# nannau/DoWnGAN

Measured on AMD Instinct MI355X. Metric: train-step samples/sec (G+D+GP), higher is better.
Workload: dtype bf16

## Files before the change

### downgan_amd/_lib.py

```python
from __future__ import annotations

import ctypes as C
import os

_HERE = os.path.dirname(os.path.abspath(__file__))
LIB_PATH = os.environ.get("DG_LIB_OVERRIDE") or os.path.join(_HERE, "csrc", "libdowngan_hip.so")

DG_F32, DG_BF16 = 0, 1
STATUS = {0: "DG_OK", -1: "DG_ERR_BAD_SHAPE", -2: "DG_ERR_BAD_DTYPE", -3: "DG_ERR_BAD_ARG", -4: "DG_ERR_LAUNCH"}


class Epilogue(C.Structure):
    _fields_ = [("bias", C.c_void_p), ("has_act", C.c_int), ("act_slope", C.c_float),
                ("r1", C.c_void_p), ("ldr1", C.c_int64), ("s1", C.c_float),
                ("r2", C.c_void_p), ("ldr2", C.c_int64), ("s2", C.c_float),
                ("mask", C.c_void_p), ("ldmask", C.c_int64), ("mask_slope", C.c_float),
                ("accumulate", C.c_int), ("mask_bits", C.c_void_p), ("out_bits", C.c_void_p),
                ("mask_c0", C.c_int), ("mask_last", C.c_int), ("out_q", C.c_void_p), ("out_qs", C.c_void_p), ("ldqs", C.c_int64),
                ("out_u", C.c_void_p), ("out_ue", C.c_void_p), ("skip_y", C.c_int), ("out_amax", C.c_void_p)]


class ConvGeom(C.Structure):
    _fields_ = [("dtype", C.c_int), ("N", C.c_int), ("H", C.c_int), ("W", C.c_int),
                ("Cin", C.c_int), ("Cout", C.c_int), ("stride", C.c_int), ("cin_real", C.c_int), ("pixel_shuffle", C.c_int),
# ... 113 lines not shown
                ("nbins", C.c_int), ("below", C.c_int * TEMPORAL_MAX_THR), ("lag", C.c_int * TEMPORAL_MAX_LAGS),
                ("scale", C.c_float * EOF_MAX_C), ("offset", C.c_float * EOF_MAX_C),
                ("thr", (C.c_float * TEMPORAL_MAX_THR) * HIST_MAX_OUT), ("lo", (C.c_float * TEMPORAL_MAX_LAGS) * HIST_MAX_OUT),
                ("inv_w", (C.c_float * TEMPORAL_MAX_LAGS) * HIST_MAX_OUT)]


MINMAX_PARTS = 256
_vp, _i, _i64, _f = C.c_void_p, C.c_int, C.c_int64, C.c_float
_PROTOS = {
    "dg_conv3x3_fwd": [C.POINTER(ConvGeom), C.POINTER(Epilogue), _vp, _vp, _vp, _vp],
    "dg_conv3x3_dgrad": [C.POINTER(ConvGeom), C.POINTER(Epilogue), _vp, _vp, _vp, _vp],
    "dg_conv3x3_wgrad": [C.POINTER(ConvGeom), _vp, _vp, _vp, _vp, _vp],
    "dg_conv3x3_wgrad_dense": [_vp, _i, _vp, _vp, _vp, _vp, _vp],
    "dg_conv3x3_wgrad_f8": [C.POINTER(ConvGeom), _vp, _vp, _vp, _vp, _vp, _vp],
    "dg_exp_from_amax": [_vp, _i, _i, _vp, _vp],
    "dg_conv3x3_wgrad_dense_f8": [C.POINTER(ConvGeom), _i, _vp, _vp, _vp, _vp, _vp, _vp],
    "dg_gather_gemm": [C.POINTER(GGDesc), C.POINTER(Epilogue), _vp, _vp, _vp, _vp],
    "dg_conv3x3_plan": [C.POINTER(ConvGeom), _i, C.POINTER(GGDesc)],
    "dg_last_conv_kernels": [],
    "dg_last_wgrad_kernel": [],
    "dg_conv3x3_dgrad_launches": [C.POINTER(ConvGeom)],
    "dg_conv3x3_dgrad_stream_eligible": [C.POINTER(ConvGeom), C.POINTER(Epilogue)],
    "dg_set_s2_dgrad_stream": [C.c_int],
    "dg_colsum": [_i, _vp, _i64, _i64, _i64, _i64, _i, _vp, _vp],
    "dg_colsum_multi": [_i, _vp, _i64, _i64, _i, _i, _vp, _vp],
    "dg_repack_conv_weights": [_i, _i, _vp, _vp, _i, _i, _vp],
    "dg_repack_dense_dgrad": [_i, _vp, _i, _i, _vp, _vp],
    "dg_wgrad_unswap": [_vp, _vp, _i, _i, _vp],
    "dg_linear_fwd": [_i, _vp, _i64, _vp, _i64, _vp, _i, _i, _i, _i64, _vp],
    "dg_linear_dx": [_i, _i, _vp, _i, _vp, _i64, _vp, _i64, _vp, _i64, _f, _i, _i, _i64, _vp],
    "dg_linear_dw": [_i, _vp, _i, _vp, _i64, _vp, _i64, _i, _i, _i64, _vp],
    "dg_linear_dw_wide": [_i, _vp, _i, _vp, _i64, _vp, _i64, _i, _i, _i64, _i, _vp],
    "dg_bias_act": [_i, _vp, _i, _vp, _vp, _i, _i, _i, _i, _f, _vp, _i, _f, _vp],
    "dg_mask_mul": [_i, _vp, _i64, _vp, _i64, _i64, _i, _f, _vp],
    "dg_axpby": [_i, _vp, _i64, _vp, _i64, _f, _vp, _i64, _f, _i64, _i, _vp],
    "dg_gp_interp": [_i, _vp, _vp, _vp, _vp, _i, _i64, _vp],
    "dg_gp_interp_c2": [_i, _vp, _vp, _i64, _vp, _vp, _vp, _vp, _i, _i64, _vp],
    "dg_scale_rows_c2": [_i, _vp, _i64, _vp, _vp, _i, _i64, _vp],
    "dg_sumsq_rows": [_i, _vp, _i, _i64, _vp, _vp],
    "dg_gp_finish": [_vp, _i, _i, _f, _f, _vp, _vp, _vp],
    "dg_scale_rows": [_i, _vp, _vp, _vp, _i, _i64, _vp],
    "dg_l1": [_i, _vp, _i64, _vp, _i64, _i64, _i, _vp, _vp, _i64, _f, _vp, _i64, _vp],
    "dg_sqdiff": [_i, _vp, _i64, _vp, _i64, _i64, _i, _vp, _vp],
    "dg_sum_strided": [_vp, _i, _i, _f, _vp, _vp],
    "dg_fill_col": [_vp, _i, _i, _i, _f, _vp],
    "dg_adam": [_vp, _vp, _vp, _vp, _vp, _i64, _f, _f, _f, _f, _i, _f, _vp],
# ... 137 lines not shown
```

### downgan_amd/csrc/conv_plan.hip

```cpp
#include "gg_common.h"

thread_local int g_last_kinds = 0;

static int gg_validate(const dg_gg_desc* d, bool f8 = false, bool compact_src = false) {
  if (d->dtype != DG_F32 && d->dtype != DG_BF16) return DG_ERR_BAD_DTYPE;
  const int epc = f8 ? 16 : d->dtype == DG_F32 ? 4 : 8;
  if (d->N <= 0 || d->Hs <= 0 || d->Ws <= 0 || d->Hg <= 0 || d->Wg <= 0 || d->Hd <= 0 || d->Wd <= 0) return DG_ERR_BAD_SHAPE;
  if (d->Cred <= 0 || d->Cred % 8 || d->Nout <= 0 || d->Nout % 16) return DG_ERR_BAD_SHAPE;
  if (d->ntaps < 1 || d->ntaps > 9) return DG_ERR_BAD_SHAPE;
  if ((compact_src ? d->lds % 2 || d->lds < 2 : d->lds % epc) || d->ldd % 4 || d->ldw % epc) return DG_ERR_BAD_SHAPE;
  for (int t = 0; t < d->ntaps; ++t) {
    if (d->tap_dy[t] < -1 || d->tap_dy[t] > 1 || d->tap_dx[t] < -1 || d->tap_dx[t] > 1) return DG_ERR_BAD_ARG;
    if (d->tap_w[t] < 0 || d->tap_w[t] > 8) return DG_ERR_BAD_ARG;
  }
  if (d->src_ps && ((d->Cred / 4) % 8)) return DG_ERR_BAD_SHAPE;
  if (d->dst_ps && ((d->Nout / 4) % 16)) return DG_ERR_BAD_SHAPE;
  if ((long long)d->N * d->Hg * d->Wg >= (1ll << 31)) return DG_ERR_BAD_SHAPE;
  if (d->dst_ps) {
    if (2 * d->Hg > d->Hd || 2 * d->Wg > d->Wd) return DG_ERR_BAD_SHAPE;
  } else {
    if ((d->Hg - 1) * d->dy_mul + d->dy_off >= d->Hd || (d->Wg - 1) * d->dx_mul + d->dx_off >= d->Wd) return DG_ERR_BAD_SHAPE;
    if (d->dy_off < 0 || d->dx_off < 0 || d->dy_mul < 1 || d->dx_mul < 1) return DG_ERR_BAD_SHAPE;
  }
  return DG_OK;
// ... 232 lines not shown
  int n = dg_conv3x3_plan(g, 1, d);
  if (n < 0) return n;
  dg_gg_desc ds;
  if (seg_dgrad_desc(d, n, &ds) && ds.Cred % 128 == 0) {
    ds.lds = q->ldxq;
    return gather_gemm_impl(&ds, ep, q->xq, q->wq, dx, stream, false, q, true);
  }
  for (int i = 0; i < n; ++i) {
    d[i].lds = q->ldxq;
    int rc = gather_gemm_impl(&d[i], ep, q->xq, q->wq, dx, stream, false, q);
    if (rc) return rc;
  }
  return DG_OK;
}

extern "C" int dg_last_conv_kernels(void) { return g_last_kinds; }

extern "C" int dg_conv3x3_dgrad_stream_eligible(const dg_conv_geom* g, const dg_epilogue* ep) {
  const int rc = geom_validate(g);
  if (rc) return rc;
  return s2dgrad_stream_eligible(g, ep) ? 1 : 0;
}

extern "C" int dg_conv3x3_dgrad_launches(const dg_conv_geom* g) {
  dg_gg_desc d[4], ds;
  const int n = dg_conv3x3_plan(g, 1, d);
  if (n < 0) return n;
  return seg_dgrad_desc(d, n, &ds) ? 1 : n;
}
```

### downgan_amd/csrc/conv_s2dgrad.hip

```cpp
#include "gg_common.h"

namespace {

constexpr int NT = 512;
constexpr int RING_PIX = 17;
constexpr int RING_PITCH = 288;
constexpr int MASK_OFF = RING_PIX * RING_PITCH;
constexpr int RING_ROW = MASK_OFF + 2 * 32 * 16;
constexpr int RING_CHUNKS = RING_PIX * 16;

struct S2DArgs {
  const char* dy; const char* w; char* dx; const char* mask_bits;
  float slope;
  int Ho, Wo;
  int nstrips, nitems, trips;
};

__device__ __forceinline__ __amdgpu_buffer_rsrc_t uniform_rsrc(const char* p) {
  const unsigned long long b = (unsigned long long)p;
  const unsigned long long u = ((unsigned long long)(unsigned)__builtin_amdgcn_readfirstlane((int)(unsigned)(b >> 32)) << 32) |
                               (unsigned)__builtin_amdgcn_readfirstlane((int)(unsigned)b);
  return __builtin_amdgcn_make_buffer_rsrc((void*)u, 0, (int)DG_OOB_OFF, 0x00020000);
}

template <bool MASK>
__device__ __forceinline__ void store_pixel(const f32x4_t& f0, const f32x4_t& f1, unsigned mb, float slope, __amdgpu_buffer_rsrc_t rY,
                                            unsigned off) {
  float v[8] = {f0[0], f0[1], f0[2], f0[3], f1[0], f1[1], f1[2], f1[3]};
  if (MASK) {
    unsigned sh = mb << 24;
    const float one = 1.f;
#pragma unroll
    for (int e = 7; e >= 0; --e) {
      float f;
      asm("v_add_co_u32_e32 %1, vcc, %1, %1\n\tv_cndmask_b32_e32 %0, %2, %3, vcc" : "=&v"(f), "+v"(sh) : "v"(slope), "v"(one) : "vcc");
      v[e] *= f;
    }
  }
  u32x4_t t;
#pragma unroll
  for (int k = 0; k < 4; ++k) t[k] = pack_bf16x2(v[2 * k], v[2 * k + 1]);
  __builtin_amdgcn_raw_buffer_store_b128(t, rY, off, 0, 0);
}

template <bool MASK, bool C11>
__device__ __forceinline__ void s2d_run(const S2DArgs& a, char* ring) {
  constexpr int NTAP = C11 ? 4 : 5;
  const int tid = threadIdx.x, lane = tid & 63, q = (tid >> 6) & 3;
  const int l15 = lane & 15, g = lane >> 4;

  uint4 wr[NTAP * 8];
  {
    constexpr int TW11[4] = {0, 2, 6, 8}, TWX[5] = {4, 3, 5, 1, 7};
#pragma unroll
    for (int cb = 0; cb < 2; ++cb)
#pragma unroll
      for (int t = 0; t < NTAP; ++t)
#pragma unroll
        for (int kk = 0; kk < 2; ++kk)
#pragma unroll
          for (int j = 0; j < 2; ++j) {
            const int n = 32 * q + 8 * (l15 >> 2) + 4 * j + (l15 & 3);
            const int tw = C11 ? TW11[t] : TWX[t];
            wr[((cb * NTAP + t) * 2 + kk) * 2 + j] =
                *reinterpret_cast<const uint4*>(a.w + ((long long)n * 1152 + tw * 128 + 64 * cb + 32 * kk + 8 * g) * 2);
          }
// ... 178 lines not shown
```

### downgan_amd/csrc/gg_common.h

```cpp
#pragma once
#include "dg_internal.h"

#include <stdlib.h>
#include <type_traits>


extern thread_local int g_last_kinds;

struct GGArgs {
  const void* x; const void* w; void* y;
  const float* bias; const void* r1; const void* r2; const void* mask;
  const void* mask_bits; void* out_bits;
  void* out_q; void* out_qs;
  void* out_u; const unsigned char* out_ue;
  int no_y;
  unsigned* out_amax;
  int ldqs, qs_shift;
  long long ldx, ldw, ldy, ldr1, ldr2, ldmask;
  int M, Hg, Wg, Hs, Ws;
  int cch, kchunks, Cred, ntaps;
  int sy_mul, sx_mul;
  unsigned long long tap_lo; unsigned tap_hi;
  int Nout, Hd, Wd, dy_mul, dx_mul, dy_off, dx_off;
  int src_ps, dst_ps, cps_src_chunks, cps_dst;
// ... 480 lines not shown
      case 2305: run(std::integral_constant<int, 2305>{}, htag); break;
      case 2312: run(std::integral_constant<int, 2312>{}, htag); break;
      case 2328: run(std::integral_constant<int, 2328>{}, htag); break;
      case 2336: run(std::integral_constant<int, 2336>{}, htag); break;
      case 258: run(std::integral_constant<int, 258>{}, htag); break;
      case 261: run(std::integral_constant<int, 261>{}, htag); break;
      case 2306: run(std::integral_constant<int, 2306>{}, htag); break;
      case 2309: run(std::integral_constant<int, 2309>{}, htag); break;
      case 4353: run(std::integral_constant<int, 4353>{}, htag); break;
      case 4354: run(std::integral_constant<int, 4354>{}, htag); break;
      case 4357: run(std::integral_constant<int, 4357>{}, htag); break;
      case 6402: run(std::integral_constant<int, 6402>{}, htag); break;
      case 6405: run(std::integral_constant<int, 6405>{}, htag); break;
      default: run(std::integral_constant<int, -1>{}, htag); break;
    }
  };
  dispatch(std::integral_constant<int, 0>{});
  EPI_STAMP(2);
  if constexpr (NH == 2) dispatch(std::integral_constant<int, 1>{});
  EPI_STAMP(3);
#undef EPI_STAMP
}

struct F8Args { const unsigned char* xs; const unsigned char* ws; int ldxs; };

int gg_launch_rows(GGArgs& a, int dtype, hipStream_t st);
bool gg_regroup_taps_by_plane(GGArgs& a);
bool gg_halo_row_step_ok(long long Ws, long long ldx, int dtype, int mult);
int gg_launch_halo(GGArgs& a, int dtype, int N, bool s2, bool ps, int nw, hipStream_t st);
int gg_launch_halo_f8(GGArgs& a, const F8Args& f, int N, bool s2, int nw, hipStream_t st);
int gg_launch_halo16(GGArgs& a, int dtype, int N, hipStream_t st);
int gg_launch_im2col(GGArgs& a, int dtype, hipStream_t st);
bool s2dgrad_stream_eligible(const dg_conv_geom* g, const dg_epilogue* ep);
int s2dgrad_stream_mode();
int s2dgrad_stream_launch(const dg_conv_geom* g, const dg_epilogue* ep, const void* dy, const void* w, void* dx, hipStream_t st);
```

### downgan_amd/engine.py

```python
from __future__ import annotations

import dataclasses
import math
import os

import torch

from . import layout
from .ops import Conv

G_SLOPE = 0.01
C_SLOPE = 0.2
RES_SCALE = 0.2
FC_HID = 100
FC_HID_P = 112
FC_HID_LD = 128
FC_OUT_P = 16


@dataclasses.dataclass
class HyperParams:
    gp_lambda: float = 10.0
    critic_iterations: int = 5
    batch_size: int = 32
# ... 132 lines not shown
        self.c_pad = [layout.pad16(c) for c in self.c_real]
        self.convs = []
        h = fine_dim
        for l, st in enumerate(self.STRIDES):
            self.convs.append(Conv(batch, h, h, self.c_pad[l], self.c_pad[l + 1], st, False,
                                   cin_real=(nc if l == 0 and nc <= 2 else 0), net="C",
                                   cin_alg=self.c_real[l], cout_alg=self.c_real[l + 1]))
            h //= st
        self.hf = h
        self.fc_k = h * h * self.c_pad[8]
        P = self.P = ParamStore(ops)
        for l, cv in enumerate(self.convs):
            P.add(f"features.{2 * l}.weight", (cv.Cout, 9, cv.Cin))
            P.conv_dgrad[f"features.{2 * l}.weight"] = (cv.Cout, cv.Cin)
        P.add("features.0.bias", (self.c_pad[1],))
        P.add("classifier.0.weight", (FC_HID_P, self.fc_k))
        P.add("classifier.0.bias", (FC_HID_LD,))
        P.add("classifier.2.weight", (FC_OUT_P, FC_HID_LD))
        P.add("classifier.2.bias", (FC_OUT_P,))
        P.finalize()
        o = ops
        use_bits = os.environ.get("DG_NO_MASK_BITS") is None and all(c >= 128 and c % 64 == 0 for c in self.c_pad[1:])
        self.f8 = bool(getattr(o, "f8", False))
        self.stacked = bool(stacked) and use_bits and not self.f8 and 3 * batch <= 128 and os.environ.get("DG_NO_FC1_FUSED") is None
        self.stack_from = (int(stacked) - 1 if (stacked is not True and int(stacked) > 1) else 0) if self.stacked else 0
        cap = 3 * batch if self.stacked else batch
        self.cap = cap
        full = lambda cv: (cap,) + tuple(o.out_shape(cv))[1:]
        self._acts_all = [o.zeros(*full(cv)) for cv in self.convs[:7]] + [None]
        self._us_all = [o.zeros(*full(cv)) for cv in self.convs]
        self._bits_all = [o.zeros(*o.bits_shape(full(cv)), dtype=torch.int16) for cv in self.convs] if use_bits else None
        self.acts = [a[:batch] if a is not None else o.zeros(*o.out_shape(self.convs[7])) for a in self._acts_all]
        self.us = [u[:batch] for u in self._us_all]
        self.act_bits = [b[:batch] for b in self._bits_all] if use_bits else None
        self._h1pre_all = o.zeros(cap, FC_HID_LD, dtype=torch.float32)
        self._h1_all = o.zeros(cap, FC_HID_LD)
        self._outpre_all = o.zeros(cap, FC_OUT_P, dtype=torch.float32)
        self._out_all = o.zeros(cap, FC_OUT_P, dtype=torch.float32)
        self._dout_all = o.zeros(cap, FC_OUT_P, dtype=torch.float32)
        self.uh1 = o.zeros(batch, FC_HID_LD, dtype=torch.float32)
        self._cv_cache = {}
        self._tan = self._th1pre = self._th1 = self._ones = None
        self.fc1_fused = 3 * batch <= 128 and os.environ.get("DG_NO_FC1_FUSED") is None
        if self.fc1_fused:
            self._y7_all = o.zeros(4 * batch, *self.acts[7].shape[1:])
            self._uh1_all = o.zeros(3 * batch, FC_HID_LD, dtype=torch.float32)
# ... 85 lines not shown
        o, P = self.ops, self.P
        if self.fc1_fused:
            s = 3 if fc1_slot is None else fc1_slot
            self.acts[7] = self._y7_all[s * self.B:(s + 1) * self.B]
        cur = x
        want_u = self.f8 and for_wgrad and self._act_exp_ok
        self._u_act_live = want_u
        l0u = self.l0u and self._act_exp_ok
        for l, cv in enumerate(self.convs):
            f8kw = dict(xq=self.actq[l - 1] if l else None, wq=self.wq_f[l], out_q=self.actq[l]) if self.f8 else {}
            if want_u and self.actu[l] is not None:
                f8kw["out_u"] = self.actu[l]
            if l0u and l == 0:
                f8kw = dict(out_u=self.actu[0], out_amax=self._a0_amax, skip_y=True)
            elif l0u and l == 1:
                f8kw["xq"] = self.actu[0]
            elif self.l0u and l == 0:
                f8kw["out_amax"] = self._a0_amax
            if not (l0u and l == 0) and self._activation_unread(l, for_wgrad):
                f8kw["skip_y"] = True
            self._act_stored[l] = not f8kw.get("skip_y", False)
            o.conv_fwd(cv, cur, P.w(f"features.{2 * l}.weight"), self.acts[l],
                       bias=P.master("features.0.bias") if l == 0 else None, act=C_SLOPE,
                       out_bits=self.act_bits[l] if self.act_bits else None, **f8kw)
            cur = self.acts[l]
        return self._head_forward(self.acts[7].view(self.B, self.fc_k), 1)

    def _activation_unread(self, l, for_wgrad):
        return bool(self.f8 and self.skip_dead and l <= 6 and self.actq[l] is not None and self.act_bits is not None
                    and (self.ops.f8_eligible(self.convs[l], "fwd") or (l == 0 and self._l0_f8_out))
                    and (not for_wgrad or (self._u_act_live and self.wg8[l + 1] and self._us_exp_ok)))

    def _head_forward(self, y7, n):
        o, P, B = self.ops, self.P, self.B
        h1pre, h1, outpre, out = (t[:n * B] for t in (self._h1pre_all, self._h1_all, self._outpre_all, self._out_all))
        passes = [slice(p * B, (p + 1) * B) for p in range(n)]
        h1pre.zero_()
        for rows in passes:
            o.linear_fwd(y7[rows], P.w2d("classifier.0.weight"), h1pre[rows], o_real=FC_HID, net="C")
        o.bias_act(h1pre, P.master("classifier.0.bias"), h1, act=C_SLOPE)
        outpre.zero_()
        for rows in passes:
            o.linear_fwd(h1[rows], P.w2d("classifier.2.weight"), outpre[rows], o_real=1, net="C")
        o.bias_act(outpre, P.master("classifier.2.bias"), out)
        return out

    def backward(self, x, dout_value, wgrad=True, dx=None, fc1_slot=None, u_role="loss"):
        o, P = self.ops, self.P
        uh1 = self.uh1 if fc1_slot is None else self._uh1_all[fc1_slot * self.B:(fc1_slot + 1) * self.B]
# ... 125 lines not shown
                                       "u_role=\"gp\" right before the tangent pass (gp_pass does)")
                o.conv_wgrad(cv, t, us[l], P.grad(name).reshape(-1))
            if self.f8 and l > 0 and self.tan_exp[l - 1] is not None and tq is not None and not (l == 1 and t0_census):
                o.block_exp_max(tq[1], self.tan_exp[l - 1])
            tn = self._tan[l & 1][:self.acts[l].numel()].view(self.acts[l].shape)
            if l == 7 and fc1_slot is not None:
                tn = self._y7_all[fc1_slot * B:(fc1_slot + 1) * B]
            f8kw, tqn = {}, None
            if self.f8:
                if self.actq[l] is not None:
                    n, sh = self.acts[l].numel(), self.acts[l].shape
                    tqn = (self._tanq[l & 1][0][:n].view(sh), self._tanq[l & 1][1][:n // 32].view(*sh[:-1], sh[-1] // 32))
                f8kw = dict(xq=tq, wq=self.wq_f[l], out_q=tqn)
            tun = None
            if self.f8 and self.tan_exp[l] is not None and tqn is not None and self._tan_exp_ok:
                tun = (self._tanu[l & 1][:self.acts[l].numel()].view(self.acts[l].shape), self.tan_exp[l])
                f8kw["out_u"] = tun
                if self._tangent_unread(l):
                    f8kw["skip_y"] = True
            if self.l0u and l == 0 and tun is not None and f8kw.get("skip_y") and r0 == 0:
                f8kw = dict(out_u=tun, out_amax=self._t0_amax, skip_y=True)
                tqn, t0_census = tun, True
            if bits:
                o.conv_fwd(cv, t, P.w(name), tn, mask_bits=bits[l], mask_slope=C_SLOPE, **f8kw)
            else:
                o.conv_fwd(cv, t, P.w(name), tn, mask=acts[l], mask_slope=C_SLOPE, **f8kw)
            if l == 1 and t0_census:
                o.exp_from_amax(self._t0_amax, self.tan_exp[0])
            t, tq, tu = tn, tqn, tun
        if self.f8 and any(e is not None for e in self.tan_exp):
            self._tan_exp_ok = True
        t7 = t.view(B, self.fc_k)
        if fc1_slot is None:
            o.linear_dw(uh1[:, :FC_HID_P], t7, P.grad("classifier.0.weight"), o_real=FC_HID, net="C")
        self._th1pre.zero_()
        o.linear_fwd(t7, P.w2d("classifier.0.weight"), self._th1pre, o_real=FC_HID, net="C")
        o.bias_act(self._th1pre, None, self._th1, mask=h1, mask_slope=C_SLOPE)
        o.linear_dw(self._ones, self._th1, P.grad("classifier.2.weight"), o_real=1, net="C")

    def _tangent_unread(self, l):
        return bool(self.skip_dead and self._bits_all is not None and l < 7 and self.wg8[l + 1] and self._us_live
                    and (self.ops.f8_eligible(self.convs[l], "fwd") or (l == 0 and self._l0_f8_out)))

    def _cvn(self, n):
        if n not in self._cv_cache:
            self._cv_cache[n] = [dataclasses.replace(cv, N=n) for cv in self.convs]
        return self._cv_cache[n]

    def forward_stacked(self, x3):
        o, P, B = self.ops, self.P, self.B
        cur = x3
        for l, cv in enumerate(self._cvn(3 * B)):
            w, bias = P.w(f"features.{2 * l}.weight"), P.master("features.0.bias") if l == 0 else None
            if l < self.stack_from:
                for p in range(3):
                    r = slice(p * B, (p + 1) * B)
                    o.conv_fwd(self.convs[l], cur[r], w, self._acts_all[l][r], bias=bias, act=C_SLOPE, out_bits=self._bits_all[l][r])
            else:
                o.conv_fwd(cv, cur, w, self._acts_all[l], bias=bias, act=C_SLOPE, out_bits=self._bits_all[l])
            cur = self._acts_all[l]
        return self._head_forward(self._acts_all[7].view(3 * B, self.fc_k), 3)

    def backward_stacked(self, x3, dout_values, dx):
        o, P, B = self.ops, self.P, self.B
        n3, w2 = 3 * B, slice(0, 2 * B)
        self._head_backward(self._acts_all[7].view(n3, self.fc_k), self._us_all[7].view(n3, self.fc_k), dout_values, 2, self._uh1_all, True)
        cv3, cv2, cv1 = self._cvn(n3), self._cvn(2 * B), self.convs
        for l in range(7, -1, -1):
            name = f"features.{2 * l}.weight"
            xin = self._acts_all[l - 1] if l > 0 else x3
            db = P.grad("features.0.bias") if l == 0 else None
            per_pass = l < self.stack_from
            if per_pass:
                for p in range(2):
                    r = slice(p * B, (p + 1) * B)
                    o.conv_wgrad(cv1[l], xin[r], self._us_all[l][r], P.grad(name).reshape(-1), db=db)
            else:
                o.conv_wgrad(cv2[l], xin[w2], self._us_all[l][w2], P.grad(name).reshape(-1), db=db)
            if l > 0 and per_pass:
                for p in range(3):
# ... 616 lines not shown
```

### downgan_amd/ops.py

```python
from __future__ import annotations

import ctypes as C
import dataclasses

import os
import torch

from . import _lib
from ._lib import ConvGeom, Epilogue, check

TORCH_DTYPE = {"f32": torch.float32, "bf16": torch.bfloat16}
DG_DTYPE = {"f32": _lib.DG_F32, "bf16": _lib.DG_BF16}


@dataclasses.dataclass(frozen=True)
class Conv:
    N: int
    H: int
    W: int
    Cin: int
    Cout: int
    stride: int = 1
    pixel_shuffle: bool = False
    cin_real: int = 0
# ... 201 lines not shown
        if skip_y:
            assert (out_q is not None or out_u is not None) and not accumulate
            ep.skip_y = 1
        if out_amax is not None:
            assert out_amax.dtype == torch.int32 and out_amax.is_cuda and out_amax.is_contiguous() and out_amax.numel() == out.shape[-1] // 32
            ep.out_amax = out_amax.data_ptr()
        return ep

    def out_shape(self, cv: Conv):
        if cv.pixel_shuffle:
            return (cv.N, 2 * cv.Ho, 2 * cv.Wo, cv.Cout // 4)
        return (cv.N, cv.Ho, cv.Wo, cv.Cout)

    def f8_eligible(self, cv: Conv, kind):
        if kind == "wgrad":
            return (self.f8 and self.f8_wgrad and cv.net == "C" and not cv.pixel_shuffle and cv.Cin % 128 == 0
                    and cv.Cout % 128 == 0 and cv.Wo % 64 == 0)
        cred, nout = (cv.Cin, cv.Cout) if kind == "fwd" else (cv.Cout, cv.Cin)
        nets = ("C", "G") if (self.f8_generator and (kind == "fwd" or self.f8_gbwd)) else ("C",)
        if self.f8_generator and self.f8_gtail and kind == "fwd" and cv.net == "T":
            return cred % 128 == 0 and nout > 64 and (not cv.pixel_shuffle or (cv.Cout // 4) % 32 == 0)
        return self.f8 and cv.net in nets and cred % 128 == 0 and nout > 64 and not cv.pixel_shuffle

    def conv_fwd(self, cv: Conv, x, w_fwd, y, xq=None, wq=None, **ep):
        self._act(x); self._act(y); self._act(w_fwd)
        assert tuple(x.shape) == (cv.N, cv.H, cv.W, cv.Cin) or (cv.cin_real and tuple(x.shape) == (cv.N, cv.H, cv.W, 2) and cv.stride == 1), (x.shape, cv)
        assert tuple(y.shape) == self.out_shape(cv), (y.shape, cv)
        assert w_fwd.numel() == cv.Cout * 9 * cv.Cin and w_fwd.is_contiguous()
        g = self._geom(cv, pix_layout(x)[0], pix_layout(y)[0])
        e = self._epilogue(y, **ep)
        if self.f8_eligible(cv, "fwd"):
            check(self._timed("conv_fwd", self.conv_flops(cv), lambda: self._conv_f8(self.lib.dg_conv3x3_fwd_f8, g, e, x, w_fwd, cv.Cout, cv.Cin, y, xq, wq),
                              self.conv_bytes(cv, ep), cv.net, self._geom_tag(cv)), "dg_conv3x3_fwd_f8")
            return
        check(self._timed("conv_fwd", self.conv_flops(cv), lambda: self.lib.dg_conv3x3_fwd(
            C.byref(g), C.byref(e), _ptr(x), _ptr(w_fwd), _ptr(y), self._stream()), self.conv_bytes(cv, ep), cv.net, self._geom_tag(cv)), "dg_conv3x3_fwd")

    def conv_dgrad(self, cv: Conv, dy, w_dgrad, dx, xq=None, wq=None, **ep):
        self._act(dy); self._act(dx); self._act(w_dgrad)
        assert tuple(dx.shape) == (cv.N, cv.H, cv.W, cv.Cin), (dx.shape, cv)
        assert tuple(dy.shape) == self.out_shape(cv), (dy.shape, cv)
        assert w_dgrad.numel() == cv.Cout * 9 * cv.Cin and w_dgrad.is_contiguous()
        g = self._geom(cv, pix_layout(dx)[0], pix_layout(dy)[0])
        e = self._epilogue(dx, **ep)
        if self.f8_eligible(cv, "dgrad"):
            check(self._timed("conv_dgrad", self.conv_flops(cv), lambda: self._conv_f8(self.lib.dg_conv3x3_dgrad_f8, g, e, dy, w_dgrad, cv.Cin, cv.Cout, dx, xq, wq),
                              self.conv_bytes(cv, ep), cv.net, self._geom_tag(cv)), "dg_conv3x3_dgrad_f8")
            return
        check(self._timed("conv_dgrad", self.conv_flops(cv), lambda: self.lib.dg_conv3x3_dgrad(
            C.byref(g), C.byref(e), _ptr(dy), _ptr(w_dgrad), _ptr(dx), self._stream()), self.conv_bytes(cv, ep), cv.net, self._geom_tag(cv)), "dg_conv3x3_dgrad")

    def quant_mxfp8(self, src, q=None, scales=None):
        Cc = src.shape[-1]
        assert Cc % 128 == 0 and src.stride(-1) == 1 and src.is_cuda and src.dtype in (torch.float32, torch.bfloat16)
        if src.dim() == 4:
            ld, rows = pix_layout(src)
# ... 745 lines not shown
```

### include/downgan_hip.h

```cpp
#ifndef DOWNGAN_HIP_H
#define DOWNGAN_HIP_H

#include <stddef.h>
#include <stdint.h>

#ifdef __cplusplus
extern "C" {
#endif

#define DG_F32 0
#define DG_BF16 1

typedef enum dg_status {
  DG_OK = 0,
  DG_ERR_BAD_SHAPE = -1,
  DG_ERR_BAD_DTYPE = -2,
  DG_ERR_BAD_ARG = -3,
  DG_ERR_LAUNCH = -4
} dg_status;

typedef struct dg_epilogue {
  const float* bias;
  int has_act;
  float act_slope;
// ... 57 lines not shown

int dg_conv3x3_wgrad_dense_f8(const dg_conv_geom* g, int nconv, const void* xq, const void* ex, const void* dyq, const void* ey,
                              float* const* dw, void* stream);

int dg_colsum(int dtype, const void* dy, int64_t rows_outer, int64_t ld_outer, int64_t rows_inner,
              int64_t ld, int C, float* db, void* stream);

int dg_colsum_multi(int dtype, const void* dy, int64_t rows, int64_t ld, int C, int nseg, float* const* db, void* stream);

int dg_gather_gemm(const dg_gg_desc* d, const dg_epilogue* ep, const void* x, const void* w, void* y,
                   void* stream);

int dg_last_conv_kernels(void);

int dg_last_wgrad_kernel(void);

int dg_conv3x3_plan(const dg_conv_geom* g, int kind, dg_gg_desc* out);

int dg_conv3x3_dgrad_launches(const dg_conv_geom* g);

int dg_conv3x3_dgrad_stream_eligible(const dg_conv_geom* g, const dg_epilogue* ep);

int dg_set_s2_dgrad_stream(int on);

int dg_repack_conv_weights(int dtype, int kind, const float* master, void* dst, int CoutP, int CinP,
                           void* stream);
int dg_repack_dense_dgrad(int dtype, const float* const* masters, int nconv, int F, void* dst, void* stream);
int dg_wgrad_unswap(const float* tmp, float* dw, int CoutP, int CinP, void* stream);


int dg_linear_fwd(int dtype, const void* x, int64_t ldx, const void* w, int64_t ldw, float* y,
                  int ldy, int B, int O, int64_t K, void* stream);
int dg_linear_dx(int dtype, int out_dtype, const float* dy, int ldo, const void* w, int64_t ldw,
                 void* dx, int64_t lddx, const void* mask, int64_t ldmask, float mask_slope, int B,
                 int O, int64_t K, void* stream);
int dg_linear_dw(int dtype, const float* dy, int ldo, const void* x, int64_t ldx, float* dw,
                 int64_t lddw, int B, int O, int64_t K, void* stream);
int dg_linear_dw_wide(int dtype, const float* dy, int ldo, const void* x, int64_t ldx, float* dw,
                      int64_t lddw, int B, int O, int64_t K, int accumulate, void* stream);


int dg_bias_act(int out_dtype, const float* in, int ldi, const float* bias, void* out, int ldo,
                int rows, int C, int has_act, float slope, const void* mask, int ldmask,
                float mask_slope, void* stream);
int dg_mask_mul(int dtype, void* u, int64_t ldu, const void* y, int64_t ldy, int64_t rows, int C,
                float slope, void* stream);
// ... 293 lines not shown
```

Measured before the change: 73.74.

## Add persistent streaming kernel for stride-2 128-channel conv forward

```diff
diff --git a/downgan_amd/_lib.py b/downgan_amd/_lib.py
--- a/downgan_amd/_lib.py
+++ b/downgan_amd/_lib.py
@@ -159,6 +159,9 @@
     "dg_conv3x3_dgrad_launches": [C.POINTER(ConvGeom)],
     "dg_conv3x3_dgrad_stream_eligible": [C.POINTER(ConvGeom), C.POINTER(Epilogue)],
     "dg_set_s2_dgrad_stream": [C.c_int],
+    "dg_conv3x3_fwd_s2_stream_eligible": [C.POINTER(ConvGeom), C.POINTER(Epilogue)],
+    "dg_conv3x3_fwd_s2_stream": [C.POINTER(ConvGeom), C.POINTER(Epilogue), _vp, _vp, _vp, _vp],
+    "dg_set_s2_fwd_stream_grid": [C.c_int],
     "dg_colsum": [_i, _vp, _i64, _i64, _i64, _i64, _i, _vp, _vp],
     "dg_colsum_multi": [_i, _vp, _i64, _i64, _i, _i, _vp, _vp],
     "dg_repack_conv_weights": [_i, _i, _vp, _vp, _i, _i, _vp],
diff --git a/downgan_amd/csrc/conv_plan.hip b/downgan_amd/csrc/conv_plan.hip
--- a/downgan_amd/csrc/conv_plan.hip
+++ b/downgan_amd/csrc/conv_plan.hip
@@ -278,6 +278,22 @@
   return s2dgrad_stream_eligible(g, ep) ? 1 : 0;
 }
 
+extern "C" int dg_conv3x3_fwd_s2_stream_eligible(const dg_conv_geom* g, const dg_epilogue* ep) {
+  const int rc = geom_validate(g);
+  if (rc) return rc;
+  return s2fwd_stream_eligible(g, ep) ? 1 : 0;
+}
+
+extern "C" int dg_conv3x3_fwd_s2_stream(const dg_conv_geom* g, const dg_epilogue* ep, const void* x, const void* w_fwd, void* y,
+                                        void* stream) {
+  g_last_kinds = 0;
+  if (!g || !x || !w_fwd || !y) return DG_ERR_BAD_ARG;
+  const int rc = geom_validate(g);
+  if (rc) return rc;
+  if (!s2fwd_stream_eligible(g, ep)) return DG_ERR_BAD_SHAPE;
+  return s2fwd_stream_launch(g, ep, x, w_fwd, y, reinterpret_cast<hipStream_t>(stream));
+}
+
 extern "C" int dg_conv3x3_dgrad_launches(const dg_conv_geom* g) {
   dg_gg_desc d[4], ds;
   const int n = dg_conv3x3_plan(g, 1, d);
diff --git a/downgan_amd/csrc/conv_s2dgrad.hip b/downgan_amd/csrc/conv_s2dgrad.hip
--- a/downgan_amd/csrc/conv_s2dgrad.hip
+++ b/downgan_amd/csrc/conv_s2dgrad.hip
@@ -15,33 +15,6 @@
   int Ho, Wo;
   int nstrips, nitems, trips;
 };
-
-__device__ __forceinline__ __amdgpu_buffer_rsrc_t uniform_rsrc(const char* p) {
-  const unsigned long long b = (unsigned long long)p;
-  const unsigned long long u = ((unsigned long long)(unsigned)__builtin_amdgcn_readfirstlane((int)(unsigned)(b >> 32)) << 32) |
-                               (unsigned)__builtin_amdgcn_readfirstlane((int)(unsigned)b);
-  return __builtin_amdgcn_make_buffer_rsrc((void*)u, 0, (int)DG_OOB_OFF, 0x00020000);
-}
-
-template <bool MASK>
-__device__ __forceinline__ void store_pixel(const f32x4_t& f0, const f32x4_t& f1, unsigned mb, float slope, __amdgpu_buffer_rsrc_t rY,
-                                            unsigned off) {
-  float v[8] = {f0[0], f0[1], f0[2], f0[3], f1[0], f1[1], f1[2], f1[3]};
-  if (MASK) {
-    unsigned sh = mb << 24;
-    const float one = 1.f;
-#pragma unroll
-    for (int e = 7; e >= 0; --e) {
-      float f;
-      asm("v_add_co_u32_e32 %1, vcc, %1, %1\n\tv_cndmask_b32_e32 %0, %2, %3, vcc" : "=&v"(f), "+v"(sh) : "v"(slope), "v"(one) : "vcc");
-      v[e] *= f;
-    }
-  }
-  u32x4_t t;
-#pragma unroll
-  for (int k = 0; k < 4; ++k) t[k] = pack_bf16x2(v[2 * k], v[2 * k + 1]);
-  __builtin_amdgcn_raw_buffer_store_b128(t, rY, off, 0, 0);
-}
 
 template <bool MASK, bool C11>
 __device__ __forceinline__ void s2d_run(const S2DArgs& a, char* ring) {
diff --git a/downgan_amd/csrc/conv_s2fwd.hip b/downgan_amd/csrc/conv_s2fwd.hip
--- /dev/null
+++ b/downgan_amd/csrc/conv_s2fwd.hip
@@ -0,0 +1,249 @@
+#include "gg_common.h"
+
+namespace {
+
+constexpr int NT = 512;
+constexpr int NODD = 17, NPIX = 33;
+constexpr int PITCH = 288;
+constexpr int ROW = NPIX * PITCH;
+constexpr int MASK_OFF = 2 * ROW;
+constexpr int PAIR = MASK_OFF + 256;
+constexpr int PSUM_OFF = 4 * PAIR;
+constexpr int LDS_BYTES = PSUM_OFF + 2 * 8192;
+
+struct S2FArgs {
+  const char* x; const char* w; char* y; const char* mask_bits; char* out_bits;
+  float act_slope, mask_slope;
+  int H, W, Ho, Wo;
+  int nstrips, nitems, trips;
+};
+
+constexpr int EP_ACT = 1, EP_MASK = 2, EP_OBITS = 4;
+
+template <int EP, bool PRE>
+__device__ __forceinline__ void s2f_run(const S2FArgs& a, char* lds) {
+  constexpr int NTAP = PRE ? 5 : 4;
+  constexpr bool MASK = (EP & EP_MASK) != 0;
+  const int tid = threadIdx.x, lane = tid & 63, q = (tid >> 6) & 3;
+  const int wave = __builtin_amdgcn_readfirstlane(tid >> 6);
+  const int l15 = lane & 15, g = lane >> 4;
+
+  uint4 wr[NTAP * 8];
+  {
+    constexpr int TWP[5] = {4, 3, 5, 1, 7}, TWS[4] = {0, 2, 6, 8};
+#pragma unroll
+    for (int t = 0; t < NTAP; ++t)
+#pragma unroll
+      for (int cb = 0; cb < 2; ++cb)
+#pragma unroll
+        for (int kk = 0; kk < 2; ++kk)
+#pragma unroll
+          for (int j = 0; j < 2; ++j) {
+            const int n = 32 * q + 8 * (l15 >> 2) + 4 * j + (l15 & 3);
+            const int tw = PRE ? TWP[t] : TWS[t];
+            wr[((t * 2 + cb) * 2 + kk) * 2 + j] =
+                *reinterpret_cast<const uint4*>(a.w + ((long long)n * 1152 + tw * 128 + 64 * cb + 32 * kk + 8 * g) * 2);
+          }
+  }
+
+  const char* const fbO = lds + l15 * PITCH + g * 16;
+  const char* const fbE = fbO + NODD * PITCH;
+  const int fk = tid >> 4;
+  char* const fill_dst = lds + ((fk & 1) ? NODD + (fk >> 1) : (fk >> 1)) * PITCH + (tid & 15) * 16;
+  const bool xwave = !PRE && wave == 4, mwave = MASK && !PRE && wave == 5;
+  const bool xfill = lane < 32, mfill = lane < 16;
+  char* const xfill_dst = lds + (lane >> 4) * ROW + 16 * PITCH + (lane & 15) * 16;
+  char* const mfill_dst = lds + MASK_OFF + lane * 16;
+  char* const psum = lds + PSUM_OFF + q * 2048 + lane * 16;
+
+  for (int trip = 0; trip < a.trips; ++trip) {
+    const int item = (int)blockIdx.x + trip * (int)gridDim.x;
+    if (item >= a.nitems) break;
+    const int img = item / a.nstrips, c0 = (item - img * a.nstrips) * 16;
+    const __amdgpu_buffer_rsrc_t rX = uniform_rsrc(a.x + (long long)img * a.H * a.W * 256);
+    const __amdgpu_buffer_rsrc_t rY = uniform_rsrc(a.y + ((long long)img * a.Ho * a.Wo + c0) * 256);
+    const __amdgpu_buffer_rsrc_t rM = uniform_rsrc(MASK ? a.mask_bits + ((long long)img * a.Ho * a.Wo + c0) * 16 : a.y);
+    const __amdgpu_buffer_rsrc_t rB = uniform_rsrc((EP & EP_OBITS) ? a.out_bits + ((long long)img * a.Ho * a.Wo + c0) * 16 : a.y);
+    const int fcol = 2 * c0 - 1 + fk;
+    const unsigned fill_off = (unsigned)fcol < (unsigned)a.W ? (unsigned)(fcol * 256 + (tid & 15) * 16) : DG_OOB_OFF;
+    const unsigned xfill_off = (xfill && 2 * c0 + 31 < a.W) ? (unsigned)(((lane >> 4) * a.W + 2 * c0 + 31) * 256 + (lane & 15) * 16) : DG_OOB_OFF;
+    const unsigned mfill_off = (mfill && c0 + lane < a.Wo) ? (unsigned)(lane * 16) : DG_OOB_OFF;
+    const unsigned rowb = (unsigned)a.W * 256u;
+    struct Staged { u32x4_t r0, r1, x, m; };
+    auto fetch_pair = [&](int p, Staged& s) {
+      const bool ok = p >= 0 && p < a.Ho;
+      const unsigned base = (unsigned)(2 * p) * rowb;
+      s.r0 = __builtin_amdgcn_raw_buffer_load_b128(rX, ok ? fill_off + base : DG_OOB_OFF, 0, 0);
+      s.r1 = __builtin_amdgcn_raw_buffer_load_b128(rX, ok ? fill_off + base + rowb : DG_OOB_OFF, 0, 0);
+      if (xwave) s.x = __builtin_amdgcn_raw_buffer_load_b128(rX, ok ? xfill_off + base : DG_OOB_OFF, 0, 0);
+      if (mwave) s.m = __builtin_amdgcn_raw_buffer_load_b128(rM, ok ? mfill_off + (unsigned)p * (unsigned)a.Wo * 16u : DG_OOB_OFF, 0, 0);
+    };
+    auto write_pair = [&](int p, const Staged& s) {
+      const int so = (p & 3) * PAIR;
+      *reinterpret_cast<uint4*>(fill_dst + so) = __builtin_bit_cast(uint4, s.r0);
+      *reinterpret_cast<uint4*>(fill_dst + so + ROW) = __builtin_bit_cast(uint4, s.r1);
+      if (xwave && xfill) *reinterpret_cast<uint4*>(xfill_dst + so) = __builtin_bit_cast(uint4, s.x);
+      if (mwave && mfill) *reinterpret_cast<uint4*>(mfill_dst + so) = __builtin_bit_cast(uint4, s.m);
+    };
+    const unsigned pix_ok = c0 + l15 < a.Wo ? 0u : DG_OOB_OFF;
+    const unsigned st_lane = pix_ok | (unsigned)(l15 * 256 + 64 * q + 16 * g);
+    const unsigned ob_lane = (g == 0 ? pix_ok : DG_OOB_OFF) | (unsigned)(l15 * 16 + 4 * q);
+    const char* const mrd = lds + MASK_OFF + l15 * 16 + 4 * q + g;
+
+    Staged st0, st1;
+    fetch_pair(-1, st0); fetch_pair(0, st1);
+    write_pair(-1, st0); write_pair(0, st1);
+    fetch_pair(1, st0);
+    __syncthreads();
+
+    auto step = [&](int r, const Staged& staged, Staged& nxt) __attribute__((always_inline)) {
+      fetch_pair(r + 2, nxt);
+      const int ro = PRE ? r : r - 1;
+      const int sP = (ro & 3) * PAIR, sM = ((ro - 1) & 3) * PAIR;
+      unsigned mb = 0u;
+      if (MASK && !PRE) mb = *reinterpret_cast<const unsigned char*>(mrd + sP);
+      __builtin_amdgcn_sched_barrier(0);
+      auto link = [&](int t, int cb, const char* fb, f32x4_t (&acc)[2]) {
+#pragma unroll
+        for (int kk = 0; kk < 2; ++kk) {
+          const uint4 b = *reinterpret_cast<const uint4*>(fb + cb * 128 + kk * 64);
+#pragma unroll
+          for (int j = 0; j < 2; ++j) Mma<bf16_t>::run(wr[((t * 2 + cb) * 2 + kk) * 2 + j], b, acc[j]);
+        }
+      };
+      if constexpr (PRE) {
+        if (r < a.Ho) {
+          f32x4_t acc[2] = {f32x4_t{0.f, 0.f, 0.f, 0.f}, f32x4_t{0.f, 0.f, 0.f, 0.f}};
+#pragma unroll
+          for (int cb = 0; cb < 2; ++cb) link(0, cb, fbE + sP, acc);
+#pragma unroll
+          for (int cb = 0; cb < 2; ++cb) {
+            link(1, cb, fbO + sP, acc); link(2, cb, fbO + sP + PITCH, acc);
+          }
+#pragma unroll
+          for (int cb = 0; cb < 2; ++cb) {
+            link(3, cb, fbE + sM + ROW, acc); link(4, cb, fbE + sP + ROW, acc);
+          }
+          char* const ps = psum + (r & 1) * 8192;
+          *reinterpret_cast<f32x4_t*>(ps) = acc[0];
+          *reinterpret_cast<f32x4_t*>(ps + 1024) = acc[1];
+        }
+      } else {
+        if (r > 0) {
+          const char* const ps = psum + (ro & 1) * 8192;
+          f32x4_t acc[2] = {*reinterpret_cast<const f32x4_t*>(ps), *reinterpret_cast<const f32x4_t*>(ps + 1024)};
+#pragma unroll
+          for (int cb = 0; cb < 2; ++cb) {
+            link(0, cb, fbO + sM + ROW, acc); link(1, cb, fbO + sM + ROW + PITCH, acc);
+            link(2, cb, fbO + sP + ROW, acc); link(3, cb, fbO + sP + ROW + PITCH, acc);
+          }
+          if constexpr ((EP & EP_ACT) != 0) {
+            if (a.act_slope >= 0.f && a.act_slope <= 1.f) {
+#pragma unroll
+              for (int j = 0; j < 2; ++j)
+#pragma unroll
+                for (int e = 0; e < 4; ++e) { const float p = acc[j][e] * a.act_slope; acc[j][e] = __builtin_fmaxf(acc[j][e], p); }
+            } else {
+#pragma unroll
+              for (int j = 0; j < 2; ++j)
+#pragma unroll
+                for (int e = 0; e < 4; ++e) acc[j][e] = leaky(acc[j][e], a.act_slope);
+            }
+          }
+          const unsigned rowo = (unsigned)ro * (unsigned)a.Wo;
+          store_pixel<MASK>(acc[0], acc[1], mb, a.mask_slope, rY, st_lane + rowo * 256u);
+          if constexpr ((EP & EP_OBITS) != 0) {
+            unsigned ob = 0;
+#pragma unroll
+            for (int k = 7; k >= 0; --k)
+              asm("v_cmp_lt_f32_e32 vcc, 0, %1\n\tv_addc_co_u32_e32 %0, vcc, %0, %0, vcc" : "+v"(ob) : "v"(acc[k >> 2][k & 3]) : "vcc");
+            ob <<= 8 * g;
+            const auto s16 = __builtin_amdgcn_permlane16_swap(ob, ob, false, false);
+            ob = s16[0] | s16[1];
+            const auto s32 = __builtin_amdgcn_permlane32_swap(ob, ob, false, false);
+            ob = s32[0] | s32[1];
+            __builtin_amdgcn_raw_buffer_store_b32(ob, rB, ob_lane + rowo * 16u, 0, 0);
+          }
+        }
+      }
+      write_pair(r + 1, staged);
+      __syncthreads();
+    };
+    for (int r = 0; r <= a.Ho; r += 2) {
+      step(r, st0, st1);
+      if (r + 1 <= a.Ho) step(r + 1, st1, st0);
+    }
+  }
+}
+
+std::atomic<int> g_grid_cap{0};
+std::atomic<int> g_cus{0};
+
+}
+
+template <int EP>
+__global__ __launch_bounds__(NT, 1) void s2fwd_stream_kernel(const S2FArgs a) {
+  extern __shared__ __attribute__((aligned(16))) char s2f_lds[];
+  if (__builtin_amdgcn_readfirstlane(threadIdx.x >> 6) < 4) s2f_run<EP, true>(a, s2f_lds);
+  else s2f_run<EP, false>(a, s2f_lds);
+}
+
+bool s2fwd_stream_eligible(const dg_conv_geom* g, const dg_epilogue* ep) {
+  if (!g || g->dtype != DG_BF16 || g->stride != 2 || g->pixel_shuffle) return false;
+  if (g->N <= 0 || g->H < 16 || g->W < 16 || ((g->H | g->W) & 1)) return false;
+  if (g->Cin != 128 || g->Cout != 128 || g->ldx != 128 || g->ldy != 128) return false;
+  if (!gg_halo_row_step_ok(g->W, g->ldx, g->dtype, 2)) return false;
+  if ((long long)g->H * g->W * 256 >= (1ll << 31)) return false;
+  if (ep) {
+    if (ep->bias || ep->r1 || ep->r2 || ep->mask || ep->accumulate || ep->mask_c0 || ep->mask_last || ep->out_q || ep->out_qs || ep->out_u ||
+        ep->out_ue || ep->skip_y || ep->out_amax)
+      return false;
+    if (ep->mask_bits && (ep->has_act || ep->out_bits)) return false;
+    if (ep->out_bits && !ep->has_act) return false;
+  }
+  return true;
+}
+
+extern "C" int dg_set_s2_fwd_stream_grid(int n) { return g_grid_cap.exchange(n < 0 ? 0 : n, std::memory_order_relaxed); }
+
+template <int EP>
+static int s2fwd_launch_ep(const S2FArgs& a, int grid, hipStream_t st) {
+  DG_SET_MAX_LDS_ONCE((&s2fwd_stream_kernel<EP>), LDS_BYTES);
+  hipLaunchKernelGGL(s2fwd_stream_kernel<EP>, dim3(grid), dim3(NT), LDS_BYTES, st, a);
+  return dg_check_launch();
+}
+
+int s2fwd_stream_launch(const dg_conv_geom* g, const dg_epilogue* ep, const void* x, const void* w, void* y, hipStream_t st) {
+  if (!x || !w || !y) return DG_ERR_BAD_ARG;
+  int cus = g_cus.load(std::memory_order_relaxed);
+  if (cus <= 0) {
+    int dev = 0;
+    if (hipGetDevice(&dev) != hipSuccess || hipDeviceGetAttribute(&cus, hipDeviceAttributeMultiprocessorCount, dev) != hipSuccess || cus <= 0)
+      return DG_ERR_LAUNCH;
+    g_cus.store(cus, std::memory_order_relaxed);
+  }
+  S2FArgs a{};
+  a.x = (const char*)x; a.w = (const char*)w; a.y = (char*)y;
+  a.mask_bits = ep ? (const char*)ep->mask_bits : nullptr;
+  a.out_bits = ep ? (char*)ep->out_bits : nullptr;
+  a.act_slope = ep ? ep->act_slope : 1.f;
+  a.mask_slope = ep ? ep->mask_slope : 1.f;
+  a.H = g->H; a.W = g->W; a.Ho = g->H / 2; a.Wo = g->W / 2;
+  a.nstrips = (a.Wo + 15) / 16;
+  const long long items = (long long)g->N * a.nstrips;
+  if (items >= (1ll << 31)) return DG_ERR_BAD_SHAPE;
+  a.nitems = (int)items;
+  const int cap = g_grid_cap.load(std::memory_order_relaxed);
+  int grid = cap > 0 && cap < cus ? cap : cus;
+  if (grid > a.nitems) grid = a.nitems;
+  a.trips = (a.nitems + grid - 1) / grid;
+  g_last_kinds |= 128;
+  const int key = (ep && ep->has_act ? EP_ACT : 0) | (a.mask_bits ? EP_MASK : 0) | (a.out_bits ? EP_OBITS : 0);
+  switch (key) {
+    case 0: return s2fwd_launch_ep<0>(a, grid, st);
+    case EP_ACT: return s2fwd_launch_ep<EP_ACT>(a, grid, st);
+    case EP_ACT | EP_OBITS: return s2fwd_launch_ep<EP_ACT | EP_OBITS>(a, grid, st);
+    case EP_MASK: return s2fwd_launch_ep<EP_MASK>(a, grid, st);
+  }
+  return DG_ERR_BAD_SHAPE;
+}
diff --git a/downgan_amd/csrc/gg_common.h b/downgan_amd/csrc/gg_common.h
--- a/downgan_amd/csrc/gg_common.h
+++ b/downgan_amd/csrc/gg_common.h
@@ -526,6 +526,33 @@
 #undef EPI_STAMP
 }
 
+__device__ __forceinline__ __amdgpu_buffer_rsrc_t uniform_rsrc(const char* p) {
+  const unsigned long long b = (unsigned long long)p;
+  const unsigned long long u = ((unsigned long long)(unsigned)__builtin_amdgcn_readfirstlane((int)(unsigned)(b >> 32)) << 32) |
+                               (unsigned)__builtin_amdgcn_readfirstlane((int)(unsigned)b);
+  return __builtin_amdgcn_make_buffer_rsrc((void*)u, 0, (int)DG_OOB_OFF, 0x00020000);
+}
+
+template <bool MASK>
+__device__ __forceinline__ void store_pixel(const f32x4_t& f0, const f32x4_t& f1, unsigned mb, float slope, __amdgpu_buffer_rsrc_t rY,
+                                            unsigned off) {
+  float v[8] = {f0[0], f0[1], f0[2], f0[3], f1[0], f1[1], f1[2], f1[3]};
+  if (MASK) {
+    unsigned sh = mb << 24;
+    const float one = 1.f;
+#pragma unroll
+    for (int e = 7; e >= 0; --e) {
+      float f;
+      asm("v_add_co_u32_e32 %1, vcc, %1, %1\n\tv_cndmask_b32_e32 %0, %2, %3, vcc" : "=&v"(f), "+v"(sh) : "v"(slope), "v"(one) : "vcc");
+      v[e] *= f;
+    }
+  }
+  u32x4_t t;
+#pragma unroll
+  for (int k = 0; k < 4; ++k) t[k] = pack_bf16x2(v[2 * k], v[2 * k + 1]);
+  __builtin_amdgcn_raw_buffer_store_b128(t, rY, off, 0, 0);
+}
+
 struct F8Args { const unsigned char* xs; const unsigned char* ws; int ldxs; };
 
 int gg_launch_rows(GGArgs& a, int dtype, hipStream_t st);
@@ -538,3 +565,5 @@
 bool s2dgrad_stream_eligible(const dg_conv_geom* g, const dg_epilogue* ep);
 int s2dgrad_stream_mode();
 int s2dgrad_stream_launch(const dg_conv_geom* g, const dg_epilogue* ep, const void* dy, const void* w, void* dx, hipStream_t st);
+bool s2fwd_stream_eligible(const dg_conv_geom* g, const dg_epilogue* ep);
+int s2fwd_stream_launch(const dg_conv_geom* g, const dg_epilogue* ep, const void* x, const void* w, void* y, hipStream_t st);
diff --git a/downgan_amd/engine.py b/downgan_amd/engine.py
--- a/downgan_amd/engine.py
+++ b/downgan_amd/engine.py
@@ -178,6 +178,7 @@
         o = ops
         use_bits = os.environ.get("DG_NO_MASK_BITS") is None and all(c >= 128 and c % 64 == 0 for c in self.c_pad[1:])
         self.f8 = bool(getattr(o, "f8", False))
+        self.s2_stream = bool(getattr(o, "s2_fwd_stream", False))
         self.stacked = bool(stacked) and use_bits and not self.f8 and 3 * batch <= 128 and os.environ.get("DG_NO_FC1_FUSED") is None
         self.stack_from = (int(stacked) - 1 if (stacked is not True and int(stacked) > 1) else 0) if self.stacked else 0
         cap = 3 * batch if self.stacked else batch
@@ -309,9 +310,12 @@
             self._act_stored[l] = not f8kw.get("skip_y", False)
             o.conv_fwd(cv, cur, P.w(f"features.{2 * l}.weight"), self.acts[l],
                        bias=P.master("features.0.bias") if l == 0 else None, act=C_SLOPE,
-                       out_bits=self.act_bits[l] if self.act_bits else None, **f8kw)
+                       out_bits=self.act_bits[l] if self.act_bits else None, **f8kw, **self._s2kw(l))
             cur = self.acts[l]
         return self._head_forward(self.acts[7].view(self.B, self.fc_k), 1)
+
+    def _s2kw(self, l):
+        return {"s2_stream": True} if l == 1 and self.s2_stream else {}
 
     def _activation_unread(self, l, for_wgrad):
         return bool(self.f8 and self.skip_dead and l <= 6 and self.actq[l] is not None and self.act_bits is not None
@@ -483,7 +487,7 @@
                 f8kw = dict(out_u=tun, out_amax=self._t0_amax, skip_y=True)
                 tqn, t0_census = tun, True
             if bits:
-                o.conv_fwd(cv, t, P.w(name), tn, mask_bits=bits[l], mask_slope=C_SLOPE, **f8kw)
+                o.conv_fwd(cv, t, P.w(name), tn, mask_bits=bits[l], mask_slope=C_SLOPE, **f8kw, **self._s2kw(l))
             else:
                 o.conv_fwd(cv, t, P.w(name), tn, mask=acts[l], mask_slope=C_SLOPE, **f8kw)
             if l == 1 and t0_census:
@@ -516,7 +520,8 @@
             if l < self.stack_from:
                 for p in range(3):
                     r = slice(p * B, (p + 1) * B)
-                    o.conv_fwd(self.convs[l], cur[r], w, self._acts_all[l][r], bias=bias, act=C_SLOPE, out_bits=self._bits_all[l][r])
+                    o.conv_fwd(self.convs[l], cur[r], w, self._acts_all[l][r], bias=bias, act=C_SLOPE, out_bits=self._bits_all[l][r],
+                               **self._s2kw(l))
             else:
                 o.conv_fwd(cv, cur, w, self._acts_all[l], bias=bias, act=C_SLOPE, out_bits=self._bits_all[l])
             cur = self._acts_all[l]
diff --git a/downgan_amd/ops.py b/downgan_amd/ops.py
--- a/downgan_amd/ops.py
+++ b/downgan_amd/ops.py
@@ -247,7 +247,9 @@
             return cred % 128 == 0 and nout > 64 and (not cv.pixel_shuffle or (cv.Cout // 4) % 32 == 0)
         return self.f8 and cv.net in nets and cred % 128 == 0 and nout > 64 and not cv.pixel_shuffle
 
-    def conv_fwd(self, cv: Conv, x, w_fwd, y, xq=None, wq=None, **ep):
+    s2_fwd_stream = True
+
+    def conv_fwd(self, cv: Conv, x, w_fwd, y, xq=None, wq=None, s2_stream=False, **ep):
         self._act(x); self._act(y); self._act(w_fwd)
         assert tuple(x.shape) == (cv.N, cv.H, cv.W, cv.Cin) or (cv.cin_real and tuple(x.shape) == (cv.N, cv.H, cv.W, 2) and cv.stride == 1), (x.shape, cv)
         assert tuple(y.shape) == self.out_shape(cv), (y.shape, cv)
@@ -257,6 +259,11 @@
         if self.f8_eligible(cv, "fwd"):
             check(self._timed("conv_fwd", self.conv_flops(cv), lambda: self._conv_f8(self.lib.dg_conv3x3_fwd_f8, g, e, x, w_fwd, cv.Cout, cv.Cin, y, xq, wq),
                               self.conv_bytes(cv, ep), cv.net, self._geom_tag(cv)), "dg_conv3x3_fwd_f8")
+            return
+        if s2_stream and self.lib.dg_conv3x3_fwd_s2_stream_eligible(C.byref(g), C.byref(e)) == 1:
+            check(self._timed("conv_fwd", self.conv_flops(cv), lambda: self.lib.dg_conv3x3_fwd_s2_stream(
+                C.byref(g), C.byref(e), _ptr(x), _ptr(w_fwd), _ptr(y), self._stream()), self.conv_bytes(cv, ep), cv.net, self._geom_tag(cv)),
+                "dg_conv3x3_fwd_s2_stream")
             return
         check(self._timed("conv_fwd", self.conv_flops(cv), lambda: self.lib.dg_conv3x3_fwd(
             C.byref(g), C.byref(e), _ptr(x), _ptr(w_fwd), _ptr(y), self._stream()), self.conv_bytes(cv, ep), cv.net, self._geom_tag(cv)), "dg_conv3x3_fwd")
diff --git a/include/downgan_hip.h b/include/downgan_hip.h
--- a/include/downgan_hip.h
+++ b/include/downgan_hip.h
@@ -103,6 +103,13 @@
 int dg_conv3x3_dgrad_stream_eligible(const dg_conv_geom* g, const dg_epilogue* ep);
 
 int dg_set_s2_dgrad_stream(int on);
+
+int dg_conv3x3_fwd_s2_stream_eligible(const dg_conv_geom* g, const dg_epilogue* ep);
+
+int dg_conv3x3_fwd_s2_stream(const dg_conv_geom* g, const dg_epilogue* ep, const void* x, const void* w_fwd, void* y,
+                             void* stream);
+
+int dg_set_s2_fwd_stream_grid(int n);
 
 int dg_repack_conv_weights(int dtype, int kind, const float* master, void* dst, int CoutP, int CinP,
                            void* stream);
```

Result: no change. 73.55 (-0.3%).
